# SerezD/vqvae-vqgan-pytorch-lightning

Hardware: AMD Instinct MI355X
Metric: images/sec/node (256x256 bs=32/GPU) VQ-VAE train step (higher is better)
Workload: dtype bf16; 1 GPU; standard_vqvae cb=1024, 256x256 bs=32/GPU (encoder+VQ+decoder fwd/bwd + AdamW); yaml=example_confs/standard_vqvae.yaml, global_batch=32, parallelism=dp1, launch=hipGraph replay (fwd+bwd) + eager all-reduce + AdamW, deterministic=False

## Files before the change

### vqvae-vqgan-pytorch-lightning_amd/csrc/api.cpp

```cpp
#include <stdint.h>
#include <new>
#include "common.h"

extern "C" {

const char* vqk_status_str(int status) {
    switch (status) {
        case VQK_OK: return "ok";
        case VQK_ERR_SHAPE: return "unsupported or inconsistent shape";
        case VQK_ERR_DTYPE: return "unsupported dtype";
        case VQK_ERR_ALIGN: return "pointer is not 16-byte aligned";
        case VQK_ERR_LAUNCH: return "kernel launch failed";
        case VQK_ERR_ARG: return "bad argument";
        case VQK_ERR_WORKSPACE: return "workspace too small";
        default: return "unknown status";
    }
}

int vqk_version(void) { return 1; }
const char* vqk_arch(void) { return "gfx950"; }

}

struct vqk_ctx {
// ... 30 lines not shown
}

extern "C" int vqk_ctx_make_current(vqk_ctx* c) {
    vqkd::current_ctx() = c;
    return VQK_OK;
}

extern "C" int vqk_ctx_set_tile_queue(vqk_ctx* c, void* ws, int64_t ws_bytes) {
    if (ws && ws_bytes < 64) return VQK_ERR_WORKSPACE;
    if (ws && (reinterpret_cast<uintptr_t>(ws) & 15)) return VQK_ERR_ALIGN;
    vqkd::DetState& d = c ? c->tq : vqkd::ctx().tq;
    d.on = ws ? 1 : 0;
    d.ws = reinterpret_cast<float*>(ws);
    d.bytes = ws ? ws_bytes : 0;
    return VQK_OK;
}

extern "C" int vqk_ctx_set_scratch(vqk_ctx* c, void* ws, int64_t ws_bytes) {
    if (ws && ws_bytes < 0) return VQK_ERR_ARG;
    if (ws && (reinterpret_cast<uintptr_t>(ws) & 15)) return VQK_ERR_ALIGN;
    vqkd::DetState& d = c ? c->scratch : vqkd::ctx().scratch;
    d.on = ws ? 1 : 0;
    d.ws = reinterpret_cast<float*>(ws);
    d.bytes = ws ? ws_bytes : 0;
    return VQK_OK;
}

extern "C" int vqk_ctx_set_deterministic(vqk_ctx* c, int on, void* ws, int64_t ws_bytes) {
    if (on && ws && ws_bytes < 0) return VQK_ERR_ARG;
    if (on && ws && (reinterpret_cast<uintptr_t>(ws) & 15)) return VQK_ERR_ALIGN;
    vqkd::DetState& d = c ? c->det : vqkd::ctx().det;
    d.on = on ? 1 : 0;
    d.ws = (on && ws) ? reinterpret_cast<float*>(ws) : nullptr;
    d.bytes = (on && ws) ? ws_bytes : 0;
    return VQK_OK;
}

extern "C" int vqk_set_tile_queue(void* ws, int64_t ws_bytes) { return vqk_ctx_set_tile_queue(nullptr, ws, ws_bytes); }
extern "C" int vqk_set_scratch(void* ws, int64_t ws_bytes) { return vqk_ctx_set_scratch(nullptr, ws, ws_bytes); }
extern "C" int vqk_set_deterministic(int on, void* ws, int64_t ws_bytes) { return vqk_ctx_set_deterministic(nullptr, on, ws, ws_bytes); }

#include <string.h>
#include <stdlib.h>
namespace vqkd {
static TuneSlot g_tune[] = {
    {"MX", 0, 0},
    {"MX_1X1", 0, 0},
    {"TW16", 0, 0},
    {"STREAM_BLOCKS", 0, 0},
    {"MX_MIN_TILES", 0, 0},
    {"FPROP_SPLITK", 0, 0},
    {"SK_BLOCKS", 0, 0},
    {"SK_MINSTEPS", 0, 0},
    {"SK_MAXMB", 0, 0},
    {"UPS_PHASE", 0, 0},
    {"WGRAD_BLOCKS", 0, 0},
    {"WGMX", 0, 0},
    {"WGRAD_GEN_BLOCKS", 0, 0},
    {"WGRAD_NO_PW16", 0, 0},
    {"WGRAD_NO_P16K", 0, 0},
    {"MX_HALF", 0, 0},
    {"MX_HALF_HW", 0, 0},
    {"UPFIRDN_TILE", 0, 0},
    {"GN_BLOCKS_REDUCE", 0, 0},
    {"GN_BLOCKS_APPLY", 0, 0},
    {"GN_NT_MB", 0, 0},
    {"GN_NO_SMALL", 0, 0},
    {"WGMX_COEF_E4", 0, 0},
    {"GN_CLUSTER_MAX_HW", 0, 0},
    {"COMM_CUS", 0, 0},
    {"MX_QUARTER", 0, 0},
    {"MX_S2", 0, 0},
    {"MX_S2_DGRAD_MIN", 0, 0},
    {"VQ_LDS", 0, 0},
    {"UPS_MERGE", 0, 0},
    {"TILE_QUEUE", 0, 0},
    {"X3_WL", 0, 0},
    {"X3_WGRAD_COEF_E4", 0, 0},
    {"X3_WGRAD_FOLD", 0, 0},
    {"X3_WGRAD_PHASE", 0, 0},
    {"X3_WGRAD_PHASE_CAP_PCT", 0, 0},
    {"X3_WGRAD_PHASE_COEF_E4", 0, 0},
    {"WGRAD_GROUP_LOAD_PCT", 0, 0},
    {"WGRAD_GROUP_MIN_PPS", 0, 0}
};
static constexpr int kTune = (int)(sizeof(g_tune) / sizeof(g_tune[0]));
TuneSlot* tune_slot(const char* name) {
    for (int i = 0; i < kTune; ++i)
        if (strcmp(g_tune[i].name, name) == 0) return &g_tune[i];
    abort();
}
}

extern "C" int vqk_set_tuning(const char* name, int value) {
    if (!name) return VQK_ERR_ARG;
    for (int i = 0; i < vqkd::kTune; ++i)
        if (strcmp(vqkd::g_tune[i].name, name) == 0) {
            __atomic_store_n(&vqkd::g_tune[i].value, value, __ATOMIC_RELAXED);
            __atomic_store_n(&vqkd::g_tune[i].is_set, 1, __ATOMIC_RELEASE);
            return VQK_OK;
        }
    return VQK_ERR_ARG;
}

extern "C" int vqk_reset_tuning(void) {
    for (int i = 0; i < vqkd::kTune; ++i) __atomic_store_n(&vqkd::g_tune[i].is_set, 0, __ATOMIC_RELAXED);
    return VQK_OK;
}

extern "C" int vqk_tuning_count(void) { return vqkd::kTune; }

extern "C" const char* vqk_tuning_name(int i) { return (i >= 0 && i < vqkd::kTune) ? vqkd::g_tune[i].name : nullptr; }
```

### vqvae-vqgan-pytorch-lightning_amd/csrc/conv.hip

```cpp
#include "conv_geom.h"
#include <type_traits>
#include <stdlib.h>
#include <math.h>

namespace {

using vqkd::ConvGeom;
using vqkd::xcd_remap;
using vqkd::pack_bf16x2;

__device__ __forceinline__ float epi_act(float v, int act) {
    if (act == 1) return tanhf(v);
    if (act == 2) return fmaxf(v, 0.0f);
    if (act == 3) return v > 0.0f ? v : 0.2f * v;
    return v;
}
__device__ __forceinline__ float epi_act_sel(float v, int act) {
    const float lo = act == 2 ? 0.0f : act == 3 ? 0.2f * v : v;
    return fmaxf(v, lo);
}


template <typename T> struct Mma;
template <> struct Mma<bf16_raw> {
// ... 1171 lines not shown
        ga.act = act;
        return vqkd::launch_conv3x3_mx(x, w, bias, res, y, zeros, ga, p.tw, st);
    }
    case FORM_STREAM_THIN: {
        ConvGeom gt = g;
        gt.tiles_n = 1;
        launch_stream<TO, 1>(p, st, x, w, bias, res, y, zeros, gt, act);
        break;
    }
    case FORM_STREAM_HALF: launch_stream<TO, 2>(p, st, x, w, bias, res, y, zeros, g, act); break;
    case FORM_STREAM_FULL: launch_stream<TO, 0>(p, st, x, w, bias, res, y, zeros, g, act); break;
    case FORM_HALO_BREG: launch_halo_breg<T, TO>(p, st, x, w, bias, res, y, zeros, g, act); break;
    case FORM_HALO_LDS:
        if (p.tw == 5) launch_halo_lds<T, TO, 5>(p, st, x, w, bias, res, y, zeros, g, act);
        else launch_halo_lds<T, TO, 4>(p, st, x, w, bias, res, y, zeros, g, act);
        break;
    case FORM_THIN_IN_BF16:
        for (int cb = 0; cb < g.cout; cb += 128) {
            if (g.cout - cb > 64)
                hipLaunchKernelGGL((conv3x3_thin_in_kernel<4>), dim3((unsigned)p.blocks), dim3(256), 4 * 32 * (4 * 64 + 8) + 4 * 128, st,
                                   (const bf16_raw*)x, (const bf16_raw*)w, bias, (bf16_raw*)y, g, act, cb);
            else
                hipLaunchKernelGGL((conv3x3_thin_in_kernel<2>), dim3((unsigned)p.blocks), dim3(256), 4 * 32 * (2 * 64 + 8) + 4 * 64, st,
                                   (const bf16_raw*)x, (const bf16_raw*)w, bias, (bf16_raw*)y, g, act, cb);
        }
        break;
    case FORM_IM2COL: launch_im2col<T, TO>(p, st, x, w, bias, res, y, zeros, g, act, nullptr); break;
    case FORM_IM2COL_SPLITK: {
        float* skws = vqkd::scratch_state().ws;
        launch_im2col<T, TO>(p, st, x, w, bias, res, y, zeros, g, act, skws);
        hipLaunchKernelGGL(conv_splitk_epilogue_kernel<TO>, dim3((unsigned)(((int64_t)g.m * g.cout / 4 + 255) / 256)), dim3(256), 0, st,
                           skws, bias, (const TO*)res, (TO*)y, g, act, p.splits);
        break;
    }
    default: return VQK_ERR_ARG;
    }
    if (hipGetLastError() != hipSuccess) return VQK_ERR_LAUNCH;
    return VQK_OK;
}

int launch_fprop_any(int dtype, int out_dtype, const void* x, const void* w, const float* bias, const void* res, void* y,
                     const void* zeros, const ConvGeom& g, int act, int wlayout, int variant, hipStream_t st) {
    if (dtype == VQK_F32 && out_dtype == VQK_F32) return launch_fprop<float, float>(x, w, bias, res, y, zeros, g, act, wlayout, variant, st);
    if (dtype == VQK_BF16 && out_dtype == VQK_BF16) return launch_fprop<bf16_raw, bf16_raw>(x, w, bias, res, y, zeros, g, act, wlayout, variant, st);
    if (dtype == VQK_BF16 && out_dtype == VQK_F32) return launch_fprop<bf16_raw, float>(x, w, bias, res, y, zeros, g, act, wlayout, variant, st);
    return VQK_ERR_DTYPE;
}

int make_geom(ConvGeom& g, int dtype, int n, int h_in, int w_in, int cin, int cout, int ksize, int ups) {
    if (dtype != VQK_F32 && dtype != VQK_BF16) return VQK_ERR_DTYPE;
    const int epc = dtype == VQK_F32 ? 4 : 8;
    if (n <= 0 || h_in <= 0 || w_in <= 0 || cin <= 0 || cout <= 0) return VQK_ERR_SHAPE;
    if (ksize != 1 && ksize != 3) return VQK_ERR_SHAPE;
    if (ups != 0 && ups != 1) return VQK_ERR_ARG;
    if (cin % epc) return VQK_ERR_SHAPE;
    g.n = n; g.h_in = h_in; g.w_in = w_in; g.h = h_in << ups; g.w = w_in << ups;
    g.cin = cin; g.cout = cout; g.ks = ksize; g.ups = ups;
    g.stride = 1; g.pad = ksize >> 1; g.zs = 0; g.vh = g.h; g.vw = g.w;
    g.acc_scale = 1.0f; g.out_gain = 1.0f; g.pool = 0; g.pool_scale = 1.0f;
    g.gn_ws = nullptr; g.gn_cpg = 0; g.gn_part_nblk = 0; g.gn_part_base = 0;
    g.act = 0; g.dy_pool = 0; g.tq = nullptr; g.tq_mode = 0; g.phase_rev = 0;
    g.ntap = ksize == 1 ? 1 : 9; g.tap_oy = g.tap_ox = 0; g.src_s = 1; g.src_a = g.src_b = 0; g.dst_s = 1; g.dst_a = g.dst_b = 0;
    g.tapw = 0; g.dst_h = g.dst_w = 0; g.s2 = 0; g.phase_mode = 0;
    g.fold = 0;
    const int64_t m = (int64_t)n * g.h * g.w;
    if (m > 0x7fffffff - 256) return VQK_ERR_SHAPE;
    g.m = (int)m;
    g.cpt = cin / epc;
    g.kchunks = ksize * ksize * g.cpt;
    g.wrow_chunks = g.kchunks; g.sub = 0;
    g.tiles_m = (g.m + 127) / 128;
    g.tiles_n = (cout + 127) / 128;
    return VQK_OK;
}

}

namespace vqkd {
int conv_make_geom(ConvGeom& g, int dtype, int n, int h_in, int w_in, int cin, int cout, int ksize, int ups) {
    return make_geom(g, dtype, n, h_in, w_in, cin, cout, ksize, ups);
}
int& conv_force_variant() { return g_force_variant; }
int& conv_wgrad_blocks() { return g_wgrad_blocks; }
}

extern "C" {

int vqk_conv_set_variant(int v) { g_force_variant = v; return VQK_OK; }
int vqk_conv_set_block_caps(int stream_blocks, int wgrad_blocks) {
    g_stream_blocks = stream_blocks; g_wgrad_blocks = wgrad_blocks;
    return VQK_OK;
}

static int conv_general(int dtype, const void* x, const void* w, const float* bias, const void* residual, void* y,
                        int out_dtype, int n, int h_in, int w_in, int cin, int cout, int ksize, int stride, int pad,
                        int mode, int h_out, int w_out, int act, float acc_scale, float out_gain, int wlayout,
                        const void* zeros, void* stream) {
    VQK_REQUIRE(x && w && y && zeros, VQK_ERR_ARG);
    VQK_REQUIRE(vqk_aligned16(x) && vqk_aligned16(w) && vqk_aligned16(zeros), VQK_ERR_ALIGN);
    VQK_REQUIRE(act >= 0 && act <= 3, VQK_ERR_ARG);
    VQK_REQUIRE(wlayout == 0 || wlayout == 1 || wlayout == 5, VQK_ERR_ARG);
    VQK_REQUIRE(mode >= 0 && mode <= 2 && (stride == 1 || stride == 2) && pad >= 0, VQK_ERR_ARG);
    ConvGeom g;
    const int rc = make_geom(g, dtype, n, h_in, w_in, cin, cout, ksize, mode ? 1 : 0);
    if (rc) return rc;
    const bool plain = stride == 1 && pad == (ksize >> 1) && mode != 2 && h_out == g.h && w_out == g.w;
    if (!plain) {
        VQK_REQUIRE(wlayout == 0, VQK_ERR_ARG);
        g.zs = mode == 2;
        g.vh = mode == 2 ? 2 * h_in - 1 : g.h;
        g.vw = mode == 2 ? 2 * w_in - 1 : g.w;
        g.stride = stride; g.pad = pad;
        VQK_REQUIRE(h_out > 0 && w_out > 0, VQK_ERR_SHAPE);
        VQK_REQUIRE((h_out - 1) * stride + ksize - pad <= g.vh + pad + stride, VQK_ERR_SHAPE);
        g.h = h_out; g.w = w_out;
        const int64_t m = (int64_t)n * h_out * w_out;
        VQK_REQUIRE(m < 0x7fffff00, VQK_ERR_SHAPE);
        g.m = (int)m;
        g.tiles_m = (g.m + 127) / 128;
    }
    g.acc_scale = acc_scale; g.out_gain = out_gain;
    hipStream_t st = vqk_stream(stream);
    if (wlayout == 5) {
        VQK_REQUIRE(plain && dtype == VQK_F32 && out_dtype == VQK_F32 && (ksize == 3 || ksize == 1), VQK_ERR_ARG);
        VQK_REQUIRE(vqk_aligned16(y) && (!residual || vqk_aligned16(residual)), VQK_ERR_ALIGN);
        return vqkd::launch_conv3x3_x3(x, w, bias, residual, y, zeros, g, act, g_stream_blocks, st);
    }
    if (mode == 2 && stride == 1 && g_force_variant != CONV_VARIANT_NO_MX) {
        int r = VQK_OK;
        for (int py = 0; py < 2 && r == VQK_OK; ++py)
            for (int px = 0; px < 2 && r == VQK_OK; ++px) {
                ConvGeom gs = g;
                gs.sub = 1; gs.sub_py = py; gs.sub_px = px;
                gs.sub_h = (g.h - py + 1) / 2; gs.sub_w = (g.w - px + 1) / 2;
                if (gs.sub_h <= 0 || gs.sub_w <= 0) continue;
                gs.nkh = gs.nkw = 0;
                for (int kk = 0; kk < ksize; ++kk) {
                    if (((py + kk - pad) & 1) == 0) gs.khl[gs.nkh++] = kk;
                    if (((px + kk - pad) & 1) == 0) gs.kwl[gs.nkw++] = kk;
                }
                if (gs.nkh == 0 || gs.nkw == 0) { gs.nkh = gs.nkw = 1; gs.khl[0] = gs.kwl[0] = 0; gs.kchunks = 0; }
                else gs.kchunks = gs.nkh * gs.nkw * gs.cpt;
                gs.m = n * gs.sub_h * gs.sub_w;
                gs.tiles_m = (gs.m + 127) / 128;
                r = launch_fprop_any(dtype, out_dtype, x, w, bias, residual, y, zeros, gs, act, 0, CONV_VARIANT_IM2COL, st);
            }
        return r;
    }
    return launch_fprop_any(dtype, out_dtype, x, w, bias, residual, y, zeros, g, act, wlayout,
                            plain ? g_force_variant : (int)CONV_VARIANT_IM2COL, st);
}

int vqk_conv2d_fprop(int dtype, const void* x, const void* w, const float* bias, const void* residual, void* y,
                     int out_dtype, int n, int h_in, int w_in, int cin, int cout, int ksize, int ups, int act,
                     int wlayout, const void* zeros, void* stream) {
    VQK_REQUIRE(ups == 0 || ups == 1, VQK_ERR_ARG);
    return conv_general(dtype, x, w, bias, residual, y, out_dtype, n, h_in, w_in, cin, cout, ksize, 1, ksize >> 1, ups,
                        h_in << ups, w_in << ups, act, 1.0f, 1.0f, wlayout, zeros, stream);
}

int vqk_conv2d_fprop_pooled(int dtype, const void* x, const void* w, const float* bias, const void* residual, void* y,
                            int n, int h_in, int w_in, int cin, int cout, int ksize, int ups, float pool_scale,
                            const void* zeros, void* stream) {
    VQK_REQUIRE(x && w && y && zeros, VQK_ERR_ARG);
    VQK_REQUIRE(vqk_aligned16(x) && vqk_aligned16(w) && vqk_aligned16(zeros) && vqk_aligned16(y), VQK_ERR_ALIGN);
    VQK_REQUIRE(dtype == VQK_BF16, VQK_ERR_DTYPE);
// ... 323 lines not shown
```

### vqvae-vqgan-pytorch-lightning_amd/csrc/conv_edge.hip

```cpp
#include "conv_geom.h"

namespace {

__device__ __forceinline__ void glds16(const void* src, char* lds_wave_base) {
    __builtin_amdgcn_global_load_lds((const VQK_GLB void*)src, (VQK_LDS void*)lds_wave_base, 16, 0, 0);
}

typedef __attribute__((ext_vector_type(8))) short s16x8;

template <int PITCH, bool SWZ>
__device__ __forceinline__ bf16x8_t tr_frag(const char* tile, int k0, int cbase, int lane) {
    const int i = lane & 15, grp = (lane >> 4) & 1, kgrp = lane >> 5;
    const int col = cbase + 16 * grp + 4 * (i & 3);
    const int row = k0 + 8 * kgrp + (i >> 2);
    const char* p0;
    if (SWZ) p0 = tile + row * PITCH + (((col >> 3) ^ ((row & 3) << 2)) << 4) + ((col & 7) << 1);
    else p0 = tile + row * PITCH + col * 2;
    const char* p1 = p0 + 4 * PITCH;
    const s16x4 lo = __builtin_amdgcn_ds_read_tr16_b64_v4i16((VQK_LDS s16x4*)p0);
    const s16x4 hi = __builtin_amdgcn_ds_read_tr16_b64_v4i16((VQK_LDS s16x4*)p1);
    const s16x8 v = {lo[0], lo[1], lo[2], lo[3], hi[0], hi[1], hi[2], hi[3]};
    return __builtin_bit_cast(bf16x8_t, v);
}

constexpr int EDGE_CW = 128;
constexpr int EDGE_PIX = 128;
constexpr int EDGE_WIDE_B = EDGE_PIX * EDGE_CW * 2;
constexpr int EDGE_IM_PITCH = 144;
constexpr int EDGE_IM_B = EDGE_PIX * EDGE_IM_PITCH;
constexpr int EDGE_STAGE = EDGE_WIDE_B + EDGE_IM_B;
constexpr int EDGE_LDS = 3 * EDGE_STAGE + 4096;
constexpr int EDGE_OUT = EDGE_CW * 72;

template <int MODE>
__global__ __launch_bounds__(256, 1) void conv3x3_wgrad_thin_kernel(const bf16_raw* __restrict__ wide,
                                                                    const bf16_raw* __restrict__ thin,
                                                                    float* __restrict__ ws, const char* __restrict__ zeros,
                                                                    int n, int h, int w) {
    extern __shared__ __attribute__((aligned(16))) char smem[];
    const int tid = threadIdx.x, lane = tid & 63;
    const int wave = __builtin_amdgcn_readfirstlane(tid >> 6);
    const int total = (int)(((int64_t)n * h * w) / EDGE_PIX);
    const int G = (int)gridDim.x, b = (int)blockIdx.x;
    const int cnt = (total - b + G - 1) / G;
    const int hw = h * w;
    constexpr int SGN = MODE == 0 ? 1 : -1;

    int s_ry[5], s_rx[5], s_ty[5], s_tx[5];
#pragma unroll
    for (int t = 0; t < 5; ++t) {
        const int q = wave + 4 * t;
        const int slot = q * 64 + lane;
        const int pl = slot / 9, tap = slot - pl * 9;
        s_ry[t] = w >= EDGE_PIX ? 0 : pl / w;
        s_rx[t] = w >= EDGE_PIX ? pl : pl - (pl / w) * w;
        s_ty[t] = SGN * (tap / 3 - 1);
        s_tx[t] = SGN * (tap - (tap / 3) * 3 - 1);
    }
    auto issue = [&](int patch, int stage) {
        char* st = smem + stage * EDGE_STAGE;
        const int64_t p0 = (int64_t)patch * EDGE_PIX;
        const int img = (int)(p0 / hw), rem = (int)(p0 - (int64_t)img * hw);
        const int y0 = rem / w, x0 = rem - y0 * w;
#pragma unroll
        for (int t = 0; t < 8; ++t) {
            const int q = wave * 8 + t;
            const int row = 4 * q + (lane >> 4), pc = lane & 15;
            const int lc = pc ^ ((row & 3) << 2);
            glds16(wide + (p0 + row) * EDGE_CW + lc * 8, st + q * 1024);
        }
        const bf16_raw* timg = thin + (int64_t)img * hw * 8;
#pragma unroll
        for (int t = 0; t < 5; ++t) {
            const int q = wave + 4 * t;
            if (q < 18) {
                const int yy = y0 + s_ry[t] + s_ty[t], xx = x0 + s_rx[t] + s_tx[t];
                const void* src = zeros;
                if ((unsigned)yy < (unsigned)h && (unsigned)xx < (unsigned)w)
                    src = timg + ((int64_t)yy * w + xx) * 8;
                glds16(src, st + EDGE_WIDE_B + q * 1024);
            } else {
                glds16(zeros, smem + 3 * EDGE_STAGE + wave * 1024);
            }
        }
    };

    f32x16 acc[3];
#pragma unroll
    for (int j = 0; j < 3; ++j)
#pragma unroll
        for (int r = 0; r < 16; ++r) acc[j][r] = 0.0f;

    if (cnt > 0) issue(b, 0);
    if (cnt > 1) issue(b + G, 1);
    for (int i = 0; i < cnt; ++i) {
        if (i + 1 < cnt) asm volatile("s_waitcnt vmcnt(13)" ::: "memory");
        else asm volatile("s_waitcnt vmcnt(0)" ::: "memory");
        __syncthreads();
        if (i + 2 < cnt) issue(b + (i + 2) * G, (i + 2) % 3);
        const char* st = smem + (i % 3) * EDGE_STAGE;
#pragma unroll
        for (int k0 = 0; k0 < EDGE_PIX; k0 += 16) {
            const bf16x8_t a = tr_frag<EDGE_CW * 2, true>(st, k0, 32 * wave, lane);
#pragma unroll
            for (int j = 0; j < 3; ++j) {
                const bf16x8_t bj = tr_frag<EDGE_IM_PITCH, false>(st + EDGE_WIDE_B, k0, 32 * j, lane);
                acc[j] = __builtin_amdgcn_mfma_f32_32x32x16_bf16(a, bj, acc[j], 0, 0, 0);
            }
        }
    }
    float* part = ws + (int64_t)b * EDGE_OUT;
#pragma unroll
    for (int j = 0; j < 3; ++j) {
        const int col = 32 * j + (lane & 31);
        if (col >= 72) continue;
        const int tap = col >> 3, t = col & 7;
#pragma unroll
        for (int r = 0; r < 16; ++r) {
            const int wc = 32 * wave + (r & 3) + 8 * (r >> 2) + 4 * (lane >> 5);
            const int idx = MODE == 0 ? (wc * 9 + tap) * 8 + t : (t * 9 + tap) * EDGE_CW + wc;
            part[idx] = acc[j][r];
        }
    }
}

__global__ __launch_bounds__(256) void wgrad_thin_reduce_kernel(const float* __restrict__ ws, float* __restrict__ dw, int blocks,
                                                                int thin_true, int thin_in) {
    __shared__ float part[16][17];
    const int o = threadIdx.x & 15, kg = threadIdx.x >> 4;
    const int i = (int)blockIdx.x * 16 + o;
    float v[16];
#pragma unroll
    for (int j = 0; j < 16; ++j) {
        const int k = kg * 16 + j;
        v[j] = k < blocks ? ws[(int64_t)k * EDGE_OUT + i] : 0.0f;
    }
    float s = 0.0f;
#pragma unroll
    for (int j = 0; j < 16; ++j) s += v[j];
    part[kg][o] = s;
    __syncthreads();
    if (threadIdx.x < 16) {
        float t = 0.0f;
#pragma unroll
        for (int g2 = 0; g2 < 16; ++g2) t += part[g2][threadIdx.x];
        const int i2 = (int)blockIdx.x * 16 + (int)threadIdx.x;
        if (thin_true >= 8) dw[i2] += t;
        else if (thin_in) { const int ci = i2 & 7; if (ci < thin_true) dw[(i2 >> 3) * thin_true + ci] += t; }
        else if (i2 < thin_true * 9 * EDGE_CW) dw[i2] += t;
    }
}


constexpr int TO_TH = 8, TO_TW = 32, TO_HW2 = TO_TW + 2, TO_HPIX = (TO_TH + 2) * TO_HW2;
constexpr int TO_PITCH = 144, TO_PIECES = 48, TO_STAGE = TO_PIECES * 1024, TO_LDS = 2 * TO_STAGE;
typedef __attribute__((ext_vector_type(4))) unsigned int eu32x4;
typedef __attribute__((ext_vector_type(2))) unsigned int eu32x2;

__global__ __launch_bounds__(256, 1) void conv3x3_thin_out_kernel(const bf16_raw* __restrict__ x, const bf16_raw* __restrict__ wgt,
                                                                  const float* __restrict__ bias, bf16_raw* __restrict__ y,
                                                                  const char* __restrict__ zeros, int n, int h, int w, int act) {
    extern __shared__ __attribute__((aligned(16))) char smem[];
    const int tid = threadIdx.x, lane = tid & 63;
    const int wave = __builtin_amdgcn_readfirstlane(tid >> 6);
    const int px = lane & 15, kq = lane >> 4;
    const int tiles_x = w / TO_TW, tiles_y = h / TO_TH;
    const int total = n * tiles_y * tiles_x;
    const int G = (int)gridDim.x, b = (int)blockIdx.x;
    const int cnt = (total - b + G - 1) / G;
    if (cnt <= 0) return;

    bf16x8_t wf[2][9][2];
#pragma unroll
    for (int hf = 0; hf < 2; ++hf)
#pragma unroll
        for (int tap = 0; tap < 9; ++tap)
#pragma unroll
            for (int ks = 0; ks < 2; ++ks) {
                eu32x4 v = {0u, 0u, 0u, 0u};
                if (px < 8) v = *reinterpret_cast<const eu32x4*>(wgt + ((int64_t)px * 9 + tap) * 128 + hf * 64 + ks * 32 + kq * 8);
                wf[hf][tap][ks] = __builtin_bit_cast(bf16x8_t, v);
            }
    float bv[4] = {0.f, 0.f, 0.f, 0.f};
    if (bias && kq < 2) {
#pragma unroll
        for (int i = 0; i < 4; ++i) bv[i] = bias[4 * kq + i];
    }

    int rel[12], flg[12];
#pragma unroll
    for (int t = 0; t < 12; ++t) {
        const int slot = (wave * 12 + t) * 64 + lane;
        const int hp = slot / 9, pc = slot - hp * 9;
        const int hy = hp / TO_HW2, hx = hp - hy * TO_HW2;
        rel[t] = (((hy - 1) * w + (hx - 1)) * 128 + pc * 8) * 2;
        flg[t] = (hy == 0 ? 1 : 0) | (hy == TO_TH + 1 ? 2 : 0) | (hx == 0 ? 4 : 0) | (hx == TO_TW + 1 ? 8 : 0) |
                 ((pc == 8 || hp >= TO_HPIX) ? 16 : 0);
    }
    struct Tile { int img, y0, x0; };
    auto tile_of = [&](int i) -> Tile {
        int t = b + i * G;
        Tile tl;
        const int txi = t % tiles_x; t /= tiles_x;
        const int tyi = t % tiles_y;
        tl.img = t / tiles_y; tl.y0 = tyi * TO_TH; tl.x0 = txi * TO_TW;
        return tl;
    };
    auto issue = [&](const Tile& tl, int hf, int stage) {
        const char* base = reinterpret_cast<const char*>(x) + ((((int64_t)tl.img * h + tl.y0) * w + tl.x0) * 128 + hf * 64) * 2;
        const int tb = (tl.y0 == 0 ? 1 : 0) | (tl.y0 + TO_TH == h ? 2 : 0) | (tl.x0 == 0 ? 4 : 0) | (tl.x0 + TO_TW == w ? 8 : 0) | 16;
        char* st = smem + stage * TO_STAGE + wave * 12 * 1024;
#pragma unroll
        for (int t = 0; t < 12; ++t) {
            const void* src = (flg[t] & tb) ? (const void*)zeros : (const void*)(base + rel[t]);
            glds16(src, st + t * 1024);
        }
    };

    f32x4 acc[4];
    Tile cur = tile_of(0);
    issue(cur, 0, 0);
    int stage = 0;
    for (int i = 0; i < cnt; ++i) {
        const Tile nxt = tile_of(i + 1 < cnt ? i + 1 : i);
#pragma unroll
        for (int hf = 0; hf < 2; ++hf) {
            asm volatile("s_waitcnt vmcnt(0)" ::: "memory");
            __syncthreads();
            if (hf == 0) issue(cur, 1, stage ^ 1);
            else if (i + 1 < cnt) issue(nxt, 0, stage ^ 1);
            const char* st = smem + stage * TO_STAGE;
            if (hf == 0) {
#pragma unroll
                for (int gq = 0; gq < 4; ++gq) acc[gq] = f32x4{0.f, 0.f, 0.f, 0.f};
            }
#pragma unroll
            for (int tap = 0; tap < 9; ++tap) {
                const int ty = tap / 3, tx = tap - ty * 3;
#pragma unroll
                for (int ks = 0; ks < 2; ++ks)
#pragma unroll
                    for (int gq = 0; gq < 4; ++gq) {
                        const int hp = (2 * wave + (gq >> 1) + ty) * TO_HW2 + 16 * (gq & 1) + px + tx;
                        const bf16x8_t bf = *reinterpret_cast<const bf16x8_t*>(st + hp * TO_PITCH + (ks * 4 + kq) * 16);
                        acc[gq] = __builtin_amdgcn_mfma_f32_16x16x32_bf16(wf[hf][tap][ks], bf, acc[gq], 0, 0, 0);
                    }
            }
            stage ^= 1;
        }
        if (kq < 2) {
#pragma unroll
            for (int gq = 0; gq < 4; ++gq) {
                float v[4];
#pragma unroll
                for (int e = 0; e < 4; ++e) {
                    v[e] = acc[gq][e] + bv[e];
                    if (act == 1) v[e] = tanhf(v[e]);
                }
                const int yy = cur.y0 + 2 * wave + (gq >> 1), xx = cur.x0 + 16 * (gq & 1) + px;
                const eu32x2 o = {vqkd::pack_bf16x2(v[0], v[1]), vqkd::pack_bf16x2(v[2], v[3])};
                *reinterpret_cast<eu32x2*>(y + (((int64_t)cur.img * h + yy) * w + xx) * 8 + 4 * kq) = o;
            }
        }
        cur = nxt;
    }
}

}

extern "C" {

int64_t vqk_conv2d_wgrad_edge_ws_bytes(void) { return (int64_t)256 * EDGE_OUT * 4; }

int vqk_conv2d_wgrad_edge(int dtype, const void* x, const void* dy, float* dw, void* ws, int64_t ws_bytes, int n, int h,
                          int w, int cin, int cout, const void* zeros, void* stream) {
    return vqk_conv2d_wgrad_edge_true(dtype, x, dy, dw, ws, ws_bytes, n, h, w, cin, cout, 8, zeros, stream);
}

int vqk_conv2d_wgrad_edge_true(int dtype, const void* x, const void* dy, float* dw, void* ws, int64_t ws_bytes, int n, int h,
                               int w, int cin, int cout, int thin_true, const void* zeros, void* stream) {
    VQK_REQUIRE(x && dy && dw && ws && zeros, VQK_ERR_ARG);
    VQK_REQUIRE(thin_true >= 1 && thin_true <= 8, VQK_ERR_ARG);
    VQK_REQUIRE(vqk_aligned16(x) && vqk_aligned16(dy) && vqk_aligned16(ws) && vqk_aligned16(zeros), VQK_ERR_ALIGN);
    VQK_REQUIRE(dtype == VQK_BF16, VQK_ERR_DTYPE);
    VQK_REQUIRE(n > 0 && h > 0 && w > 0, VQK_ERR_SHAPE);
    const bool first = cin == 8 && cout == EDGE_CW, last = cout == 8 && cin == EDGE_CW;
    const int64_t m = (int64_t)n * h * w;
    VQK_REQUIRE((first || last) && ((int64_t)h * w) % EDGE_PIX == 0 && (w % EDGE_PIX == 0 || EDGE_PIX % w == 0) && m < 0x7fffffffLL,
                VQK_ERR_SHAPE);
    const int total = (int)(m / EDGE_PIX);
    int blocks = total < 256 ? total : 256;
    VQK_REQUIRE(ws_bytes >= (int64_t)blocks * EDGE_OUT * 4, VQK_ERR_ARG);
    hipStream_t st = vqk_stream(stream);
    if (first) {
        static const hipError_t attr = hipFuncSetAttribute((const void*)conv3x3_wgrad_thin_kernel<0>,
                                                           hipFuncAttributeMaxDynamicSharedMemorySize, EDGE_LDS);
        if (attr != hipSuccess) return VQK_ERR_LAUNCH;
        hipLaunchKernelGGL(conv3x3_wgrad_thin_kernel<0>, dim3((unsigned)blocks), dim3(256), EDGE_LDS, st, (const bf16_raw*)dy,
                           (const bf16_raw*)x, (float*)ws, (const char*)zeros, n, h, w);
    } else {
        static const hipError_t attr = hipFuncSetAttribute((const void*)conv3x3_wgrad_thin_kernel<1>,
                                                           hipFuncAttributeMaxDynamicSharedMemorySize, EDGE_LDS);
        if (attr != hipSuccess) return VQK_ERR_LAUNCH;
        hipLaunchKernelGGL(conv3x3_wgrad_thin_kernel<1>, dim3((unsigned)blocks), dim3(256), EDGE_LDS, st, (const bf16_raw*)x,
                           (const bf16_raw*)dy, (float*)ws, (const char*)zeros, n, h, w);
    }
    VQK_CHECK_LAUNCH();
    static_assert(EDGE_OUT % 16 == 0, "reduce blocks own 16 outputs");
    hipLaunchKernelGGL(wgrad_thin_reduce_kernel, dim3(EDGE_OUT / 16), dim3(256), 0, st, (const float*)ws, dw, blocks, thin_true, first ? 1 : 0);
    VQK_CHECK_LAUNCH();
    return VQK_OK;
}

int vqk_conv2d_thin_out(int dtype, const void* x, const void* w, const float* bias, void* y, int n, int h, int wd, int cin,
                        int cout, int act, const void* zeros, void* stream) {
    VQK_REQUIRE(x && w && y && zeros, VQK_ERR_ARG);
    VQK_REQUIRE(vqk_aligned16(x) && vqk_aligned16(w) && vqk_aligned16(y) && vqk_aligned16(zeros), VQK_ERR_ALIGN);
    VQK_REQUIRE(dtype == VQK_BF16, VQK_ERR_DTYPE);
    VQK_REQUIRE(act == 0 || act == 1, VQK_ERR_ARG);
    VQK_REQUIRE(n > 0 && cin == 128 && cout == 8 && h > 0 && wd > 0 && (h % TO_TH) == 0 && (wd % TO_TW) == 0 &&
                (int64_t)n * h * wd * 128 * 2 < 0x7fffffff0LL, VQK_ERR_SHAPE);
    const int total = n * (h / TO_TH) * (wd / TO_TW);
    const int blocks = total < 256 ? total : 256;
    static const hipError_t attr = hipFuncSetAttribute((const void*)conv3x3_thin_out_kernel,
                                                       hipFuncAttributeMaxDynamicSharedMemorySize, TO_LDS);
    if (attr != hipSuccess) return VQK_ERR_LAUNCH;
    hipLaunchKernelGGL(conv3x3_thin_out_kernel, dim3((unsigned)blocks), dim3(256), TO_LDS, vqk_stream(stream), (const bf16_raw*)x,
                       (const bf16_raw*)w, bias, (bf16_raw*)y, (const char*)zeros, n, h, wd, act);
    VQK_CHECK_LAUNCH();
    return VQK_OK;
}

}
```

### vqvae-vqgan-pytorch-lightning_amd/csrc/conv_geom.h

```cpp
#pragma once
#include "common.h"

namespace vqkd {

struct ConvGeom {
    int n, h_in, w_in, h, w, cin, cout, ks, ups;
    int stride, pad, zs, vh, vw;
    float acc_scale, out_gain;
    int pool;
    float pool_scale;
    int m;
    int sub, sub_py, sub_px, sub_h, sub_w, nkh, nkw, khl[2], kwl[2];
    int wrow_chunks;
    int cpt;
    int kchunks;
    int tiles_m, tiles_n;
    double* gn_ws;
    int gn_cpg;
    int gn_part_nblk, gn_part_base;
    int ntap, tap_oy, tap_ox, src_s, src_a, src_b, dst_s, dst_a, dst_b;
    int tapw, dst_h, dst_w, s2;
    int phase_mode;
    int phase_rev;
    int dy_pool;
    int act;
    int* tq;
    int tq_mode;
    int fold;
};

__device__ __forceinline__ int xcd_remap(int bid, int total) {
    const int q = total >> 3, r = total & 7, xcd = bid & 7, k = bid >> 3;
    return (xcd < r ? xcd * (q + 1) : r * (q + 1) + (xcd - r) * q) + k;
}

__device__ __forceinline__ unsigned pack_bf16x2(float a, float b) {
    typedef __attribute__((ext_vector_type(2))) float f32x2;
    typedef __attribute__((ext_vector_type(2))) __bf16 bf16x2_t;
    const f32x2 v = {a, b};
    return __builtin_bit_cast(unsigned, __builtin_convertvector(v, bf16x2_t));
}

int launch_conv3x3_mx(const void* x, const void* w, const float* bias, const void* res, void* y, const void* zeros,
                      const ConvGeom& g, int twlog, hipStream_t st);

int conv_make_geom(ConvGeom& g, int dtype, int n, int h_in, int w_in, int cin, int cout, int ksize, int ups);
}
enum ConvVariant : int {
    CONV_VARIANT_AUTO = -1,
    CONV_VARIANT_IM2COL = 0,
    CONV_VARIANT_HALO = 1,
    CONV_VARIANT_PLAIN_WEIGHTS = 2,
    CONV_VARIANT_BREG = 3,
    CONV_VARIANT_NO_HALF = 4,
    CONV_VARIANT_NO_MX = 5,
    CONV_VARIANT_MX = 6,
};
namespace vqkd {
int& conv_force_variant();
int& conv_wgrad_blocks();

bool conv3x3_x3_serves(const ConvGeom& g);
int launch_conv3x3_x3(const void* x, const void* w, const float* bias, const void* res, void* y, const void* zeros,
                      const ConvGeom& g, int act, int blocks_cap, hipStream_t st);
int launch_conv3x3_wgrad_x3(const void* x, const void* dy, float* dw, const ConvGeom& g, int blocks_cap, hipStream_t st);

int launch_conv3x3_thin_out_f32(const float* x, const float* w, const float* bias, const float* res, float* y, int n, int h, int wd,
                                int cin, int act, float acc_scale, float out_gain, hipStream_t st);
int launch_conv3x3_thin_in_f32(const float* x, const float* w, const float* bias, float* y, int n, int h, int wd, int cout, hipStream_t st);
int thin_wgrad_rows(int h, int w);
int launch_conv3x3_wgrad_thin_f32(int mode, const float* wide, const float* thin, float* dw, int n, int h, int w, int cw, float scale,
                                  hipStream_t st);

int launch_conv3x3_wgrad_mx(const void* x, const void* dy, float* dw, const void* zeros, const ConvGeom& g, int tiles,
                            int splits, int pps, hipStream_t st, float* part = nullptr);

#define VQK_WGRAD_GROUP_MAX 16
struct WgradGroupLayer {
    const void* x; const void* dy; float* dw;
    int n, h, w, cin, cout;
    float scale;
    int blk0, tiles, pps;
    int own;
};
struct WgradGroupTable {
    int n_layers, pad_;
    WgradGroupLayer layer[VQK_WGRAD_GROUP_MAX];
};
int launch_conv3x3_wgrad_mx_group(const WgradGroupTable& tb, int blocks, const void* zeros, hipStream_t st);

}
```

### vqvae-vqgan-pytorch-lightning_amd/ops.py

```python
from __future__ import annotations

import ctypes
import os
import threading
import weakref

import numpy as _np
import torch

from . import _native

F32, BF16 = 0, 1
_CL = torch.channels_last


def dcode(dtype: torch.dtype) -> int:
    if dtype == torch.float32:
        return F32
    if dtype == torch.bfloat16:
        return BF16
    raise RuntimeError(f'vqk: unsupported dtype {dtype}')


def epc(dtype: torch.dtype) -> int:
# ... 1415 lines not shown
            if y is not None:
                _note_presummed(y, next_gn)
        if (y is None and next_gn and k == 3 and act == 0 and layout == 0 and cin == 8 and cout_pad == o and res is None and not ups
                and out_dtype == dt):
            y = raw_conv_thin_in_gnstats(x, wq, b32, cout_pad, next_gn)
            if y is not None:
                _note_presummed(y, next_gn)
        if y is None:
            y = raw_conv_fprop(x, wq, b32, res, k, ups, act, out_dtype, cout_pad, layout)
        ctx.save_for_backward(x, weight, y if act == 1 else None)
        ctx.bias_ref, ctx.weight_ref = bias, weight
        ctx.cfg = (k, ups, act, o, i, cin, cout_pad, bias is not None, residual is not None, dt)
        ctx.phase = phase
        ctx.x3 = X3
        if (bias is not None and act == 0 and cout_pad == o and out_dtype == dt and gn_colsum_ok(y.shape[2], y.shape[3])
                and direct_grad(bias) is not None):
            _note_bias_colsum(y, bias)
        return y

    @staticmethod
    def backward(ctx, dy):
        x, weight, y = ctx.saved_tensors
        k, ups, act, o, i, cin, cout_pad, has_bias, has_res, dt = ctx.cfg
        dy = nhwc(dy)
        if dy.shape[2] * dy.shape[3] > WGRAD_GROUP_MAX_HW and _WGRAD_PENDING and wgrads_pending(x.device):
            flush_wgrads(x.device)
        if act == 1:
            d2 = torch.empty_like(dy, memory_format=_CL)
            _native.check(_native.lib().vqk_tanh_backward(dcode(dy.dtype), dy.data_ptr(), y.data_ptr(), d2.data_ptr(),
                                                          dy.numel(), _stream()), 'tanh_backward')
            dy = d2
        dres = dy if has_res else None
        dyc = dy if dy.dtype == dt else nhwc(dy.to(dt))
        dx = dw = db = None
        if ctx.needs_input_grad[0]:
            n_img, _, h_out, w_out = dyc.shape
            layout = weight_layout(dt, n_img, h_out, w_out, cout_pad, cin, k, False, x3=ctx.x3)
            if ups and ctx.phase and UPS_PHASE == 1:
                dx = raw_conv_ups_phase(dyc, packed_weight(weight, cin, cout_pad, dt, k, True, phase_layout(dt, ctx.x3)), None, cin, True)
            if dx is not None:
                pass
            elif ups and can_pool_epilogue(dt, cin, layout):
                wt = packed_weight(weight, cin, cout_pad, dt, k, True, layout)
                dx = raw_conv_fprop_pooled(dyc, wt, None, None, k, False, cin, 1.0)
            else:
                wt = packed_weight(weight, cin, cout_pad, dt, k, True, layout)
                dx = raw_conv_fprop(dyc, wt, None, None, k, False, 0, dt, cin, layout)
                if ups:
                    dx = raw_pool(dx, 1.0)
        padded = cin != i or cout_pad != o
        if ctx.needs_input_grad[1]:
            tgt = None if padded else direct_grad(ctx.weight_ref)
            thin = 8
            if padded and edge_wgrad_served(x, dyc, k, ups) and (cin == i or cout_pad == o):
                tgt = direct_grad(ctx.weight_ref)
                thin = (i if cin != i else o) if tgt is not None else 8
            if thin == 8 and wgrad_group_deferrable(x, dyc, tgt, ctx.x3, k, ups):
                defer_wgrad(x, dyc, tgt)
            else:
                dw = raw_conv_wgrad(x, dyc, k, ups, out=tgt, thin_true=thin, x3=ctx.x3)
            if tgt is not None:
                dw = None
            elif padded:
                dw = dw[:o, :i]
        if has_bias and ctx.needs_input_grad[2] and id(ctx.bias_ref) in _DB_DONE:
            _DB_DONE.discard(id(ctx.bias_ref))
        elif has_bias and ctx.needs_input_grad[2]:
            n, c, h, w = dyc.shape
            tgt = direct_grad(ctx.bias_ref) if (cout_pad == c) else None
            db = raw_colsum(n * h * w, c, dyc, out=tgt, lead=o if tgt is not None else None)
            db = None if tgt is not None else db[:o]
        return dx, dw, db, dres, None, None, None, None


def conv2d(x, weight, bias=None, residual=None, ups: bool = False, act: int = 0, out_dtype=None, next_gn: int = 0):
    return Conv2dFn.apply(x, weight, bias, residual, ups, act, out_dtype, next_gn)


class GroupNormSiLUFn(torch.autograd.Function):

    @staticmethod
    def forward(ctx, x, weight, bias, groups: int, eps: float, silu: bool):
        _require_gpu(x)
        x = nhwc(x)
        w = weight.detach().reshape(-1).contiguous()
        b = bias.detach().reshape(-1).contiguous()
        y, stats = raw_gn_forward(x, w, b, groups, eps, silu)
        ctx.save_for_backward(x, stats, w, b)
        ctx.params = (weight, bias)
        ctx.cfg = (groups, silu, weight.shape, bias.shape)
        ctx.cluster_ok = cluster_owner_ok()
        return y

    @staticmethod
    def backward(ctx, dy):
        x, stats, w, b = ctx.saved_tensors
        groups, silu, wshape, bshape = ctx.cfg
        tw, tb = direct_grad(ctx.params[0]), direct_grad(ctx.params[1])
        direct = tw is not None and tb is not None
        dx, dw, db = raw_gn_backward(x, stats, w, b, nhwc(dy), groups, silu, tw if direct else None,
                                     tb if direct else None, cluster_ok=ctx.cluster_ok)
        if direct:
            return dx, None, None, None, None, None
        return dx, dw.view(wshape), db.view(bshape), None, None, None


POOLED_BWD = _native.switch('VQK_POOLED_BWD', '1') != '0'
OVERLAP_WGRAD = _native.switch('VQK_OVERLAP_WGRAD', '1') == '1'
OVERLAP_STREAM_BLOCKS = int(_native.switch('VQK_OVERLAP_STREAM_BLOCKS', '512'))
OVERLAP_WGRAD_BLOCKS = int(_native.switch('VQK_OVERLAP_WGRAD_BLOCKS', '320'))
OVERLAP_WGRAD_BLOCKS_HI = int(_native.switch('VQK_OVERLAP_WGRAD_BLOCKS_HI', '256'))
OVERLAP_WGRAD_BLOCKS_LO = int(_native.switch('VQK_OVERLAP_WGRAD_BLOCKS_LO', str(OVERLAP_WGRAD_BLOCKS)))
OVERLAP_WGRAD_BLOCKS_MID = int(_native.switch('VQK_OVERLAP_WGRAD_BLOCKS_MID', str(OVERLAP_WGRAD_BLOCKS)))
_SIDE_STREAMS: dict = {}


def _side_stream(device) -> torch.cuda.Stream:
    st = _SIDE_STREAMS.get(device)
    if st is None:
        st = _SIDE_STREAMS[device] = torch.cuda.Stream(device=device)
    return st


def aux_stream(device, tag: str) -> torch.cuda.Stream:
    st = _SIDE_STREAMS.get((device, tag))
    if st is None:
        st = _SIDE_STREAMS[(device, tag)] = torch.cuda.Stream(device=device)
    return st


def _on_side(main, side, launch) -> None:
    fork = torch.cuda.Event()
    fork.record(main)
    side.wait_event(fork)
    with torch.cuda.stream(side):
        launch()


def _wgrad_cap(hw: int) -> int:
    if hw <= 1024:
        return OVERLAP_WGRAD_BLOCKS_LO
    return OVERLAP_WGRAD_BLOCKS_HI if hw >= 65536 else OVERLAP_WGRAD_BLOCKS_MID if hw >= 16384 else OVERLAP_WGRAD_BLOCKS


WGRAD_GROUP_MAX_HW = int(_native.switch('VQK_WGRAD_GROUP_MAX_HW', '1024'))
_WGRAD_GROUP_ITEMS = 16
_WGRAD_PENDING: dict = {}


def wgrads_pending(device=None) -> int:
    st = _WGRAD_PENDING.get(torch.cuda.current_device() if device is None else torch.device(device).index)
    return len(st['items']) if st else 0


def drop_pending_wgrads(device=None) -> None:
    st = _WGRAD_PENDING.get(torch.cuda.current_device() if device is None else torch.device(device).index)
    if st:
        st['items'].clear()
        st['task'] = -1


def _forget_stale_wgrads(device) -> None:
    if _WGRAD_PENDING and torch._C._current_graph_task_id() == -1 and wgrads_pending(device):
        drop_pending_wgrads(device)


def wgrad_group_deferrable(x, dy, target, x3: bool = False, ksize: int = 3, ups: bool = False) -> bool:
    n, cin, h, w = x.shape
    return (WGRAD_GROUP_MAX_HW > 0 and target is not None and not x3 and not DETERMINISTIC and _WGMX_ON and ksize == 3 and not ups
            and x.dtype == torch.bfloat16 and dy.dtype == torch.bfloat16 and h * w <= WGRAD_GROUP_MAX_HW and h % 8 == 0
            and w % 16 == 0 and cin % 64 == 0 and dy.shape[1] % 64 == 0 and tuple(dy.shape[2:]) == (h, w))


def defer_wgrad(x, dy, target) -> None:
    dev = x.device.index
    st = _WGRAD_PENDING.get(dev)
    if st is None:
        st = _WGRAD_PENDING[dev] = {'items': [], 'stream': None, 'task': -1}
    st['items'].append((x, dy, target))
    st['stream'] = torch.cuda.current_stream(x.device)
    task = torch._C._current_graph_task_id()
    if task != -1 and st['task'] != task:
        st['task'] = task
        torch.autograd.Variable._execution_engine.queue_callback(lambda: flush_wgrads(dev))
# ... 343 lines not shown
```

Measured before the change: 1167 images/sec.

## Software-pipeline edge wgrad LDS reads, add 3-stage thin-out option, fuse GN bias colsum

```diff
diff --git a/vqvae-vqgan-pytorch-lightning_amd/csrc/api.cpp b/vqvae-vqgan-pytorch-lightning_amd/csrc/api.cpp
--- a/vqvae-vqgan-pytorch-lightning_amd/csrc/api.cpp
+++ b/vqvae-vqgan-pytorch-lightning_amd/csrc/api.cpp
@@ -136,7 +136,9 @@
     {"X3_WGRAD_PHASE_CAP_PCT", 0, 0},
     {"X3_WGRAD_PHASE_COEF_E4", 0, 0},
     {"WGRAD_GROUP_LOAD_PCT", 0, 0},
-    {"WGRAD_GROUP_MIN_PPS", 0, 0}
+    {"WGRAD_GROUP_MIN_PPS", 0, 0},
+    {"EDGE_OUT_STAGES", 0, 0},
+    {"EDGE_WGRAD_SPAN", 0, 0}
 };
 static constexpr int kTune = (int)(sizeof(g_tune) / sizeof(g_tune[0]));
 TuneSlot* tune_slot(const char* name) {
diff --git a/vqvae-vqgan-pytorch-lightning_amd/csrc/conv.hip b/vqvae-vqgan-pytorch-lightning_amd/csrc/conv.hip
--- a/vqvae-vqgan-pytorch-lightning_amd/csrc/conv.hip
+++ b/vqvae-vqgan-pytorch-lightning_amd/csrc/conv.hip
@@ -1277,6 +1277,7 @@
 }
 int& conv_force_variant() { return g_force_variant; }
 int& conv_wgrad_blocks() { return g_wgrad_blocks; }
+int& conv_stream_blocks() { return g_stream_blocks; }
 }
 
 extern "C" {
diff --git a/vqvae-vqgan-pytorch-lightning_amd/csrc/conv_edge.hip b/vqvae-vqgan-pytorch-lightning_amd/csrc/conv_edge.hip
--- a/vqvae-vqgan-pytorch-lightning_amd/csrc/conv_edge.hip
+++ b/vqvae-vqgan-pytorch-lightning_amd/csrc/conv_edge.hip
@@ -9,18 +9,33 @@
 typedef __attribute__((ext_vector_type(8))) short s16x8;
 
 template <int PITCH, bool SWZ>
-__device__ __forceinline__ bf16x8_t tr_frag(const char* tile, int k0, int cbase, int lane) {
+__device__ __forceinline__ const char* tr_addr(const char* tile, int k0, int cbase, int lane) {
     const int i = lane & 15, grp = (lane >> 4) & 1, kgrp = lane >> 5;
     const int col = cbase + 16 * grp + 4 * (i & 3);
     const int row = k0 + 8 * kgrp + (i >> 2);
-    const char* p0;
-    if (SWZ) p0 = tile + row * PITCH + (((col >> 3) ^ ((row & 3) << 2)) << 4) + ((col & 7) << 1);
-    else p0 = tile + row * PITCH + col * 2;
+    if (SWZ) return tile + row * PITCH + (((col >> 3) ^ ((row & 3) << 2)) << 4) + ((col & 7) << 1);
+    return tile + row * PITCH + col * 2;
+}
+__device__ __forceinline__ bf16x8_t tr_join(s16x4 lo, s16x4 hi) {
+    const s16x8 v = {lo[0], lo[1], lo[2], lo[3], hi[0], hi[1], hi[2], hi[3]};
+    return __builtin_bit_cast(bf16x8_t, v);
+}
+template <int PITCH, bool SWZ>
+__device__ __forceinline__ bf16x8_t tr_frag(const char* tile, int k0, int cbase, int lane) {
+    const char* p0 = tr_addr<PITCH, SWZ>(tile, k0, cbase, lane);
     const char* p1 = p0 + 4 * PITCH;
     const s16x4 lo = __builtin_amdgcn_ds_read_tr16_b64_v4i16((VQK_LDS s16x4*)p0);
     const s16x4 hi = __builtin_amdgcn_ds_read_tr16_b64_v4i16((VQK_LDS s16x4*)p1);
-    const s16x8 v = {lo[0], lo[1], lo[2], lo[3], hi[0], hi[1], hi[2], hi[3]};
-    return __builtin_bit_cast(bf16x8_t, v);
+    return tr_join(lo, hi);
+}
+__device__ __forceinline__ void tr_read(s16x4& lo, s16x4& hi, const char* p0, int pitch4) {
+    asm volatile("ds_read_b64_tr_b16 %0, %1" : "=v"(lo) : "v"((VQK_LDS const char*)p0) : "memory");
+    asm volatile("ds_read_b64_tr_b16 %0, %1" : "=v"(hi) : "v"((VQK_LDS const char*)(p0 + pitch4)) : "memory");
+}
+template <int N>
+__device__ __forceinline__ void tr_wait(s16x4 (&f)[8]) {
+    asm volatile("s_waitcnt lgkmcnt(%8)" : "+v"(f[0]), "+v"(f[1]), "+v"(f[2]), "+v"(f[3]), "+v"(f[4]), "+v"(f[5]), "+v"(f[6]), "+v"(f[7])
+                 : "n"(N) : "memory");
 }
 
 constexpr int EDGE_CW = 128;
@@ -32,7 +47,7 @@
 constexpr int EDGE_LDS = 3 * EDGE_STAGE + 4096;
 constexpr int EDGE_OUT = EDGE_CW * 72;
 
-template <int MODE>
+template <int MODE, bool SPAN>
 __global__ __launch_bounds__(256, 1) void conv3x3_wgrad_thin_kernel(const bf16_raw* __restrict__ wide,
                                                                     const bf16_raw* __restrict__ thin,
                                                                     float* __restrict__ ws, const char* __restrict__ zeros,
@@ -96,9 +111,39 @@
     for (int i = 0; i < cnt; ++i) {
         if (i + 1 < cnt) asm volatile("s_waitcnt vmcnt(13)" ::: "memory");
         else asm volatile("s_waitcnt vmcnt(0)" ::: "memory");
-        __syncthreads();
+        if (SPAN) {
+            asm volatile("s_waitcnt lgkmcnt(0)" ::: "memory");
+            __builtin_amdgcn_s_barrier();
+        } else {
+            __syncthreads();
+        }
         if (i + 2 < cnt) issue(b + (i + 2) * G, (i + 2) % 3);
         const char* st = smem + (i % 3) * EDGE_STAGE;
+        if (SPAN) {
+            s16x4 f[2][8];
+            auto reads = [&](int k0, s16x4 (&o)[8]) {
+                tr_read(o[0], o[1], tr_addr<EDGE_CW * 2, true>(st, k0, 32 * wave, lane), 4 * EDGE_CW * 2);
+#pragma unroll
+                for (int j = 0; j < 3; ++j)
+                    tr_read(o[2 + 2 * j], o[3 + 2 * j], tr_addr<EDGE_IM_PITCH, false>(st + EDGE_WIDE_B, k0, 32 * j, lane), 4 * EDGE_IM_PITCH);
+            };
+            reads(0, f[0]);
+#pragma unroll
+            for (int ks = 0; ks < EDGE_PIX / 16; ++ks) {
+                s16x4 (&cur)[8] = f[ks & 1];
+                if (ks + 1 < EDGE_PIX / 16) {
+                    reads(16 * (ks + 1), f[(ks + 1) & 1]);
+                    tr_wait<8>(cur);
+                } else {
+                    tr_wait<0>(cur);
+                }
+                const bf16x8_t a = tr_join(cur[0], cur[1]);
+#pragma unroll
+                for (int j = 0; j < 3; ++j)
+                    acc[j] = __builtin_amdgcn_mfma_f32_32x32x16_bf16(a, tr_join(cur[2 + 2 * j], cur[3 + 2 * j]), acc[j], 0, 0, 0);
+            }
+            continue;
+        }
 #pragma unroll
         for (int k0 = 0; k0 < EDGE_PIX; k0 += 16) {
             const bf16x8_t a = tr_frag<EDGE_CW * 2, true>(st, k0, 32 * wave, lane);
@@ -153,10 +198,11 @@
 
 
 constexpr int TO_TH = 8, TO_TW = 32, TO_HW2 = TO_TW + 2, TO_HPIX = (TO_TH + 2) * TO_HW2;
-constexpr int TO_PITCH = 144, TO_PIECES = 48, TO_STAGE = TO_PIECES * 1024, TO_LDS = 2 * TO_STAGE;
+constexpr int TO_PITCH = 144, TO_PIECES = 48, TO_STAGE = TO_PIECES * 1024;
 typedef __attribute__((ext_vector_type(4))) unsigned int eu32x4;
 typedef __attribute__((ext_vector_type(2))) unsigned int eu32x2;
 
+template <int STAGES>
 __global__ __launch_bounds__(256, 1) void conv3x3_thin_out_kernel(const bf16_raw* __restrict__ x, const bf16_raw* __restrict__ wgt,
                                                                   const float* __restrict__ bias, bf16_raw* __restrict__ y,
                                                                   const char* __restrict__ zeros, int n, int h, int w, int act) {
@@ -220,15 +266,25 @@
     f32x4 acc[4];
     Tile cur = tile_of(0);
     issue(cur, 0, 0);
+    if (STAGES == 3) issue(cur, 1, 1);
     int stage = 0;
     for (int i = 0; i < cnt; ++i) {
         const Tile nxt = tile_of(i + 1 < cnt ? i + 1 : i);
 #pragma unroll
         for (int hf = 0; hf < 2; ++hf) {
-            asm volatile("s_waitcnt vmcnt(0)" ::: "memory");
-            __syncthreads();
-            if (hf == 0) issue(cur, 1, stage ^ 1);
-            else if (i + 1 < cnt) issue(nxt, 0, stage ^ 1);
+            if (STAGES == 3) {
+                if (hf == 1 && i + 1 >= cnt) asm volatile("s_waitcnt vmcnt(0)" ::: "memory");
+                else if (i == 0) asm volatile("s_waitcnt vmcnt(12)" ::: "memory");
+                else asm volatile("s_waitcnt vmcnt(16)" ::: "memory");
+                asm volatile("s_waitcnt lgkmcnt(0)" ::: "memory");
+                __builtin_amdgcn_s_barrier();
+                if (i + 1 < cnt) issue(nxt, hf, stage == 0 ? 2 : stage - 1);
+            } else {
+                asm volatile("s_waitcnt vmcnt(0)" ::: "memory");
+                __syncthreads();
+                if (hf == 0) issue(cur, 1, stage ^ 1);
+                else if (i + 1 < cnt) issue(nxt, 0, stage ^ 1);
+            }
             const char* st = smem + stage * TO_STAGE;
             if (hf == 0) {
 #pragma unroll
@@ -246,7 +302,7 @@
                         acc[gq] = __builtin_amdgcn_mfma_f32_16x16x32_bf16(wf[hf][tap][ks], bf, acc[gq], 0, 0, 0);
                     }
             }
-            stage ^= 1;
+            stage = STAGES == 3 ? (stage == 2 ? 0 : stage + 1) : stage ^ 1;
         }
         if (kq < 2) {
 #pragma unroll
@@ -290,21 +346,21 @@
                 VQK_ERR_SHAPE);
     const int total = (int)(m / EDGE_PIX);
     int blocks = total < 256 ? total : 256;
+    const int cap = vqkd::conv_wgrad_blocks();
+    if (cap > 0 && cap < blocks) blocks = cap;
     VQK_REQUIRE(ws_bytes >= (int64_t)blocks * EDGE_OUT * 4, VQK_ERR_ARG);
     hipStream_t st = vqk_stream(stream);
-    if (first) {
-        static const hipError_t attr = hipFuncSetAttribute((const void*)conv3x3_wgrad_thin_kernel<0>,
-                                                           hipFuncAttributeMaxDynamicSharedMemorySize, EDGE_LDS);
-        if (attr != hipSuccess) return VQK_ERR_LAUNCH;
-        hipLaunchKernelGGL(conv3x3_wgrad_thin_kernel<0>, dim3((unsigned)blocks), dim3(256), EDGE_LDS, st, (const bf16_raw*)dy,
-                           (const bf16_raw*)x, (float*)ws, (const char*)zeros, n, h, w);
-    } else {
-        static const hipError_t attr = hipFuncSetAttribute((const void*)conv3x3_wgrad_thin_kernel<1>,
-                                                           hipFuncAttributeMaxDynamicSharedMemorySize, EDGE_LDS);
-        if (attr != hipSuccess) return VQK_ERR_LAUNCH;
-        hipLaunchKernelGGL(conv3x3_wgrad_thin_kernel<1>, dim3((unsigned)blocks), dim3(256), EDGE_LDS, st, (const bf16_raw*)x,
-                           (const bf16_raw*)dy, (float*)ws, (const char*)zeros, n, h, w);
-    }
+    const bool span = VQK_TUNE("EDGE_WGRAD_SPAN", 1) != 0;
+#define VQK_EDGE_WGRAD(MODE, SPAN, WIDE, THIN) do { \
+        static const hipError_t attr = hipFuncSetAttribute((const void*)conv3x3_wgrad_thin_kernel<MODE, SPAN>, \
+                                                           hipFuncAttributeMaxDynamicSharedMemorySize, EDGE_LDS); \
+        if (attr != hipSuccess) return VQK_ERR_LAUNCH; \
+        hipLaunchKernelGGL((conv3x3_wgrad_thin_kernel<MODE, SPAN>), dim3((unsigned)blocks), dim3(256), EDGE_LDS, st, \
+                           (const bf16_raw*)(WIDE), (const bf16_raw*)(THIN), (float*)ws, (const char*)zeros, n, h, w); \
+    } while (0)
+    if (first) { if (span) VQK_EDGE_WGRAD(0, true, dy, x); else VQK_EDGE_WGRAD(0, false, dy, x); }
+    else { if (span) VQK_EDGE_WGRAD(1, true, x, dy); else VQK_EDGE_WGRAD(1, false, x, dy); }
+#undef VQK_EDGE_WGRAD
     VQK_CHECK_LAUNCH();
     static_assert(EDGE_OUT % 16 == 0, "reduce blocks own 16 outputs");
     hipLaunchKernelGGL(wgrad_thin_reduce_kernel, dim3(EDGE_OUT / 16), dim3(256), 0, st, (const float*)ws, dw, blocks, thin_true, first ? 1 : 0);
@@ -321,12 +377,20 @@
     VQK_REQUIRE(n > 0 && cin == 128 && cout == 8 && h > 0 && wd > 0 && (h % TO_TH) == 0 && (wd % TO_TW) == 0 &&
                 (int64_t)n * h * wd * 128 * 2 < 0x7fffffff0LL, VQK_ERR_SHAPE);
     const int total = n * (h / TO_TH) * (wd / TO_TW);
-    const int blocks = total < 256 ? total : 256;
-    static const hipError_t attr = hipFuncSetAttribute((const void*)conv3x3_thin_out_kernel,
-                                                       hipFuncAttributeMaxDynamicSharedMemorySize, TO_LDS);
-    if (attr != hipSuccess) return VQK_ERR_LAUNCH;
-    hipLaunchKernelGGL(conv3x3_thin_out_kernel, dim3((unsigned)blocks), dim3(256), TO_LDS, vqk_stream(stream), (const bf16_raw*)x,
-                       (const bf16_raw*)w, bias, (bf16_raw*)y, (const char*)zeros, n, h, wd, act);
+    int blocks = total < 256 ? total : 256;
+    const int cap = vqkd::conv_stream_blocks();
+    if (cap > 0 && cap < blocks) blocks = cap;
+    const int stages = VQK_TUNE("EDGE_OUT_STAGES", 2);
+    VQK_REQUIRE(stages == 2 || stages == 3, VQK_ERR_ARG);
+#define VQK_THIN_OUT(STAGES) do { \
+        static const hipError_t attr = hipFuncSetAttribute((const void*)conv3x3_thin_out_kernel<STAGES>, \
+                                                           hipFuncAttributeMaxDynamicSharedMemorySize, STAGES * TO_STAGE); \
+        if (attr != hipSuccess) return VQK_ERR_LAUNCH; \
+        hipLaunchKernelGGL(conv3x3_thin_out_kernel<STAGES>, dim3((unsigned)blocks), dim3(256), STAGES * TO_STAGE, vqk_stream(stream), \
+                           (const bf16_raw*)x, (const bf16_raw*)w, bias, (bf16_raw*)y, (const char*)zeros, n, h, wd, act); \
+    } while (0)
+    if (stages == 3) VQK_THIN_OUT(3); else VQK_THIN_OUT(2);
+#undef VQK_THIN_OUT
     VQK_CHECK_LAUNCH();
     return VQK_OK;
 }
diff --git a/vqvae-vqgan-pytorch-lightning_amd/csrc/conv_geom.h b/vqvae-vqgan-pytorch-lightning_amd/csrc/conv_geom.h
--- a/vqvae-vqgan-pytorch-lightning_amd/csrc/conv_geom.h
+++ b/vqvae-vqgan-pytorch-lightning_amd/csrc/conv_geom.h
@@ -59,6 +59,7 @@
 namespace vqkd {
 int& conv_force_variant();
 int& conv_wgrad_blocks();
+int& conv_stream_blocks();
 
 bool conv3x3_x3_serves(const ConvGeom& g);
 int launch_conv3x3_x3(const void* x, const void* w, const float* bias, const void* res, void* y, const void* zeros,
diff --git a/vqvae-vqgan-pytorch-lightning_amd/ops.py b/vqvae-vqgan-pytorch-lightning_amd/ops.py
--- a/vqvae-vqgan-pytorch-lightning_amd/ops.py
+++ b/vqvae-vqgan-pytorch-lightning_amd/ops.py
@@ -1521,6 +1521,7 @@
     @staticmethod
     def forward(ctx, x, weight, bias, groups: int, eps: float, silu: bool):
         _require_gpu(x)
+        ctx.db_param = _claim_bias_colsum(x)
         x = nhwc(x)
         w = weight.detach().reshape(-1).contiguous()
         b = bias.detach().reshape(-1).contiguous()
@@ -1537,8 +1538,13 @@
         groups, silu, wshape, bshape = ctx.cfg
         tw, tb = direct_grad(ctx.params[0]), direct_grad(ctx.params[1])
         direct = tw is not None and tb is not None
+        cs = None
+        if ctx.db_param is not None and gn_colsum_ok(x.shape[2], x.shape[3]) and not torch.is_grad_enabled():
+            cs = direct_grad(ctx.db_param)
+            if cs is not None:
+                _DB_DONE.add(id(ctx.db_param))
         dx, dw, db = raw_gn_backward(x, stats, w, b, nhwc(dy), groups, silu, tw if direct else None,
-                                     tb if direct else None, cluster_ok=ctx.cluster_ok)
+                                     tb if direct else None, dx_colsum=cs, cluster_ok=ctx.cluster_ok)
         if direct:
             return dx, None, None, None, None, None
         return dx, dw.view(wshape), db.view(bshape), None, None, None
```

Result: no change. 1177 images/sec, median of 6 (+0.9%).
